# dmMaze/comic-text-detector

Measured on NVIDIA H100. Metric: pages/sec @1024x1024 synthetic, higher is better.
Workload: dtype fp16

## Files before the change

comic-text-detector_b200/csrc/conv_tc.cu:

```cuda
#include <cstdlib>
#include <cstring>
#include <cuda.h>
#include <cuda_fp16.h>
#include <cuda_runtime.h>

#include "kernels.h"
#include "ptx.cuh"

namespace ctd {

constexpr int kTileW = 16;
constexpr int kThreads = 384;

template <int BN, int TH>
struct TcCfg {
  static constexpr int kABytes = TH * kTileW * 128;
  static constexpr int kBBytes = BN * 128;
  static constexpr int kStages = TH == 8 ? (BN >= 128 ? 5 : (BN >= 64 ? 8 : 10))
                                         : (BN >= 128 ? 3 : (BN >= 64 ? 4 : (BN >= 32 ? 5 : 6)));
  static constexpr int kBoxN = BN < 64 ? BN : 64;
  static constexpr int kBoxBytes = 8 * TH * kBoxN * 2;
  static constexpr int kStgBytes = (BN / kBoxN) * kBoxBytes;
  static constexpr int kBiasFloats = 512;
  static constexpr size_t kSmem = 1024 + size_t(kStages) * (kABytes + kBBytes) + 2 * kStgBytes + 256 + kBiasFloats * 4;
// ... 61 lines not shown
  }
}

template <int ACT>
__device__ __forceinline__ void epi_pair_f32(float v0, float v1, const float* __restrict__ bias_s, int col,
                                             float* __restrict__ out, int ncols, bool residual) {
  if (col >= ncols) return;
  float f0 = apply_act_precise<ACT>(v0 + bias_s[col]);
  float f1 = apply_act_precise<ACT>(v1 + bias_s[col + 1]);
  if (col + 1 < ncols) {
    if (residual) {
      const float2 r = *reinterpret_cast<const float2*>(out + col);
      f0 += r.x;
      f1 += r.y;
    }
    *reinterpret_cast<float2*>(out + col) = make_float2(f0, f1);
  } else {
    if (residual) f0 += out[col];
    out[col] = f0;
  }
}

template <int BN, int ACT>
__device__ __forceinline__ void epilogue_f32(const float (&acc)[BN / 2], const float* __restrict__ bias_s,
                                             float* const (&out)[2], const bool (&valid)[2], int ncols, int lane,
                                             bool residual) {
#pragma unroll
  for (int h = 0; h < 2; ++h) {
    if (!valid[h]) continue;
#pragma unroll
    for (int j = 0; j < BN / 8; ++j)
      epi_pair_f32<ACT>(acc[j * 4 + 2 * h], acc[j * 4 + 2 * h + 1], bias_s, j * 8 + (lane & 3) * 2, out[h], ncols,
                        residual);
  }
}

template <int BN, int TH>
__global__ void __launch_bounds__(kThreads, 1) conv_tc_kernel(const __grid_constant__ ConvTcParams p) {
  using Cfg = TcCfg<BN, TH>;
  constexpr int MT = TH / 8;
  extern __shared__ __align__(1024) uint8_t smem_tc[];
  const uint32_t raw_base = smem_u32(smem_tc);
  const uint32_t smem_base = (raw_base + 1023u) & ~1023u;
  uint8_t* const smem_gen = smem_tc + (smem_base - raw_base);
  const uint32_t a_base = smem_base;
  const uint32_t b_base = a_base + Cfg::kStages * Cfg::kABytes;
  const uint32_t stg_base = b_base + Cfg::kStages * Cfg::kBBytes;
  const uint32_t bar_base = stg_base + 2 * Cfg::kStgBytes;
  const uint32_t full_bar = bar_base, empty_bar = bar_base + 8 * Cfg::kStages, res_bar0 = bar_base + 16 * Cfg::kStages;
  float* bias_s = reinterpret_cast<float*>(smem_gen + (bar_base - smem_base) + 256);

  const int warp = threadIdx.x >> 5, lane = threadIdx.x & 31;
  const ConvGeom& g = p.g;

  const int kb = p.kb_elems;
  const uint32_t row_bytes = kb * 2;
  const uint32_t stage_tx = uint32_t(TH * kTileW) * row_bytes + uint32_t(BN) * row_bytes;
  int kblocks_per_tap = 0;
  for (int s = 0; s < g.n_src; ++s) kblocks_per_tap += p.src_kblocks[s];
  const int n_terms = p.split ? 3 : 1;
  const int its_per_tile = g.taps * kblocks_per_tap * n_terms;
  const int tiles_per_img = p.tiles_x * p.tiles_y;
  const int n_nblk = g.cout_pad / BN;
  const int spatial_tiles = g.n_img * tiles_per_img;
  const int total_tiles = spatial_tiles * n_nblk * g.n_phase;

// ... 43 lines not shown
                const int stage = it % Cfg::kStages;
                const uint32_t par = ((it / Cfg::kStages) & 1) ^ 1;
                mbar_wait_relaxed(empty_bar + 8 * stage, par);
                mbar_arrive_expect_tx(full_bar + 8 * stage, stage_tx);
                tma_load_4d(a_base + stage * Cfg::kABytes, &p.a_map[s][q], full_bar + 8 * stage, cb * kb, x0 + dx,
                            y0 + dy, img + (term == 1 ? p.split_img_off : 0));
                tma_load_2d(b_base + stage * Cfg::kBBytes, &p.b_map, full_bar + 8 * stage, kglob + cb * kb,
                            phase * g.cout_pad + nblk * BN + (term == 2 ? p.split_row_off : 0));
              }
            }
            kglob += g.src_c[s];
          }
        }
      }
    }
    return;
  }

  if constexpr (TH == 16) setmaxnreg_inc<232>();
  const int wg = (warp >> 2) - 1;
  const int wrow = ((warp & 3) << 4) + (lane >> 2);
  const bool wg_leader = (threadIdx.x & 127) == 0;
  const uint64_t a_desc0 = make_kmajor_desc(a_base + uint32_t(wg * MT) * 64u * row_bytes, row_bytes);
  const uint64_t b_desc0 = make_kmajor_desc(b_base, row_bytes);
  const uint64_t a_mstep = (64u * row_bytes) >> 4;
  const int ksteps = kb / 16;
  int stage = 0;
  uint32_t full_par = 0;
  constexpr int R = BN / 2;
  const bool nhwc16 = p.dst != nullptr && !p.split;
  const bool res16 = nhwc16 && g.residual != 0;
  const uint32_t stg = stg_base + uint32_t(wg) * Cfg::kStgBytes;
  const uint32_t res_bar = res_bar0 + 8u * uint32_t(wg);
  const uint32_t epi_bar = 1 + wg;
  uint32_t res_par = 0;

  for (int t = blockIdx.x; t < total_tiles; t += gridDim.x) {
    int phase, nblk, img, y0, x0;
    decode(t, phase, nblk, img, y0, x0);
    const int sy0 = y0 + wg * (TH / 2);
    if (res16 && wg_leader) {
      tma_store_wait_read();
      mbar_arrive_expect_tx(res_bar, Cfg::kStgBytes);
#pragma unroll
      for (int b = 0; b < BN / Cfg::kBoxN; ++b)
        tma_load_4d(stg + b * Cfg::kBoxBytes, &p.d_map[phase], res_bar, nblk * BN + b * Cfg::kBoxN, x0, sy0, img);
    }
    float acc[MT][R];
#pragma unroll
    for (int m = 0; m < MT; ++m)
#pragma unroll
      for (int i = 0; i < R; ++i) acc[m][i] = 0.f;

    bool split_done = false;
    if constexpr (BN <= 64 && TH == 8) {
      if (p.split) {
        float cross[R], tmp[R];
#pragma unroll
        for (int i = 0; i < R; ++i) cross[i] = 0.f;
        bool cross_started = false;
        for (int k_it = 0; k_it < its_per_tile; ++k_it) {
          mbar_wait(full_bar + 8 * stage, full_par);
          const uint64_t ad = a_desc0 + uint64_t(stage) * (Cfg::kABytes >> 4);
          const uint64_t bd = b_desc0 + uint64_t(stage) * (Cfg::kBBytes >> 4);
          if (k_it % 3 == 0) {
            for (int ks = 0; ks < ksteps; ++ks) {
              wgmma_fence();
              wgmma_bn<BN>(tmp, ad + 2 * ks, bd + 2 * ks, 0u);
              wgmma_commit();
              wgmma_wait<0>();
              wgmma_fence_regs(tmp);
#pragma unroll
              for (int i = 0; i < R; ++i) acc[0][i] = __fadd_rn(acc[0][i], tmp[i]);
            }
          } else {
            wgmma_fence();
            for (int ks = 0; ks < ksteps; ++ks)
              wgmma_bn<BN>(cross, ad + 2 * ks, bd + 2 * ks, (cross_started || ks > 0) ? 1u : 0u);
            wgmma_commit();
            wgmma_wait<0>();
// ... 3 lines not shown
          if (wg_leader) mbar_arrive(empty_bar + 8 * stage);
          if (++stage == Cfg::kStages) { stage = 0; full_par ^= 1u; }
        }
#pragma unroll
        for (int i = 0; i < R; ++i) acc[0][i] = __fadd_rn(acc[0][i], cross[i] * kSplitLoUnscale);
        split_done = true;
      }
    }
    if (!split_done) {
      int prev = -1;
      for (int k_it = 0; k_it < its_per_tile; ++k_it) {
        mbar_wait(full_bar + 8 * stage, full_par);
        const uint64_t ad = a_desc0 + uint64_t(stage) * (Cfg::kABytes >> 4);
        const uint64_t bd = b_desc0 + uint64_t(stage) * (Cfg::kBBytes >> 4);
        wgmma_fence();
        for (int ks = 0; ks < ksteps; ++ks)
#pragma unroll
          for (int m = 0; m < MT; ++m)
            wgmma_bn<BN>(acc[m], ad + m * a_mstep + 2 * ks, bd + 2 * ks, (k_it > 0 || ks > 0) ? 1u : 0u);
        wgmma_commit();
        wgmma_wait<1>();
        if (prev >= 0 && wg_leader) mbar_arrive(empty_bar + 8 * prev);
        prev = stage;
        if (++stage == Cfg::kStages) { stage = 0; full_par ^= 1u; }
      }
      wgmma_wait<0>();
#pragma unroll
      for (int m = 0; m < MT; ++m) wgmma_fence_regs(acc[m]);
      if (prev >= 0 && wg_leader) mbar_arrive(empty_bar + 8 * prev);
    }

    const float* bias_t = bias_s + nblk * BN;
    if (nhwc16) {
      if (res16) {
        mbar_wait(res_bar, res_par);
        res_par ^= 1u;
      } else {
        if (wg_leader) tma_store_wait_read();
        named_barrier_sync(epi_bar, 128);
      }
#define CTD_EPI(ACT)                                                                                   \
  _Pragma("unroll") for (int m = 0; m < MT; ++m) {                                                     \
    if (res16) stage_f16<BN, TH, ACT, true>(acc[m], bias_t, stg, m, warp & 3, lane);                   \
    else stage_f16<BN, TH, ACT, false>(acc[m], bias_t, stg, m, warp & 3, lane);                        \
  }
      switch (g.act) {
        case CTD_ACT_SILU: CTD_EPI(CTD_ACT_SILU) break;
        case CTD_ACT_LEAKY: CTD_EPI(CTD_ACT_LEAKY) break;
        case CTD_ACT_RELU: CTD_EPI(CTD_ACT_RELU) break;
        case CTD_ACT_SIGMOID: CTD_EPI(CTD_ACT_SIGMOID) break;
        default: CTD_EPI(CTD_ACT_NONE) break;
      }
#undef CTD_EPI
      fence_proxy_async();
      named_barrier_sync(epi_bar, 128);
      if (wg_leader) {
#pragma unroll
        for (int b = 0; b < BN / Cfg::kBoxN; ++b)
          tma_store_4d(&p.d_map[phase], stg + b * Cfg::kBoxBytes, nblk * BN + b * Cfg::kBoxN, x0, sy0, img);
        tma_store_commit();
      }
      if (p.dst_map_cols < g.cout && p.dst_map_cols < (nblk + 1) * BN) {
#pragma unroll
        for (int m = 0; m < MT; ++m)
#pragma unroll
          for (int h = 0; h < 2; ++h) {
            const int row = (wg * MT + m) * 64 + wrow + 8 * h;
            const int gy = y0 + row / kTileW, gx = x0 + row % kTileW;
            if (gy >= g.gh || gx >= g.gw) continue;
            const int oy = gy * g.out_mul + (phase >> 1), ox = gx * g.out_mul + (phase & 1);
            __half* out = p.dst + (size_t(img) * g.dst_h * g.dst_w + size_t(oy) * g.dst_w + ox) * g.dst_cstride +
                          g.dst_coff;
#pragma unroll
            for (int i = 0; i < R; ++i) {
              if (((i >> 1) & 1) != h) continue;
              const int c = (i >> 2) * 8 + (lane & 3) * 2 + (i & 1), col = nblk * BN + c;
              if (col < p.dst_map_cols || col >= g.cout) continue;
              float f;
              switch (g.act) {
                case CTD_ACT_SILU: f = apply_act<CTD_ACT_SILU>(acc[m][i] + bias_t[c]); break;
                case CTD_ACT_LEAKY: f = apply_act<CTD_ACT_LEAKY>(acc[m][i] + bias_t[c]); break;
                case CTD_ACT_RELU: f = apply_act<CTD_ACT_RELU>(acc[m][i] + bias_t[c]); break;
                case CTD_ACT_SIGMOID: f = apply_act<CTD_ACT_SIGMOID>(acc[m][i] + bias_t[c]); break;
                default: f = acc[m][i] + bias_t[c]; break;
              }
              if (res16) f = __fadd_rn(f, __half2float(out[col]));
              out[col] = __float2half_rn(f);
            }
          }
      }
      continue;
    }
    const int ph_y = phase >> 1, ph_x = phase & 1;
    const int ncols = g.cout - nblk * BN;
#pragma unroll
    for (int m = 0; m < MT; ++m) {
      int gy[2], gx[2];
      bool valid[2];
      size_t pix[2];
#pragma unroll
      for (int h = 0; h < 2; ++h) {
        const int row = (wg * MT + m) * 64 + wrow + 8 * h;
        gy[h] = y0 + row / kTileW;
        gx[h] = x0 + row % kTileW;
        valid[h] = gy[h] < g.gh && gx[h] < g.gw;
        const int oy = gy[h] * g.out_mul + ph_y, ox = gx[h] * g.out_mul + ph_x;
        pix[h] = valid[h] ? size_t(img) * g.dst_h * g.dst_w + size_t(oy) * g.dst_w + ox : 0;
      }
      if (p.dst == nullptr) {
        const int no = 5 + p.nc;
        float* rows = p.blks + (size_t(img) * p.blks_rows_per_img + p.level_row0) * no;
#pragma unroll
        for (int h = 0; h < 2; ++h) {
          if (!valid[h]) continue;
#pragma unroll
          for (int i = 0; i < R; ++i) {
            if (((i >> 1) & 1) != h) continue;
            const int c = (i >> 2) * 8 + (lane & 3) * 2 + (i & 1);
            if (c >= ncols) continue;
            const int col = nblk * BN + c;
            const int a = col / no, o = col - a * no;
            const float s = 1.0f / (1.0f + expf(-(acc[m][i] + bias_t[c])));
            float r;
            if (o == 0) r = (s * 2.0f - 0.5f + float(gx[h])) * p.det_stride;
            else if (o == 1) r = (s * 2.0f - 0.5f + float(gy[h])) * p.det_stride;
            else if (o == 2) r = (s * 2.0f) * (s * 2.0f) * p.anchor_wh[2 * a];
            else if (o == 3) r = (s * 2.0f) * (s * 2.0f) * p.anchor_wh[2 * a + 1];
            else r = s;
            rows[(size_t(a) * g.gh * g.gw + size_t(gy[h]) * g.gw + gx[h]) * no + o] = r;
          }
        }
      } else {
        float* out32[2];
#pragma unroll
        for (int h = 0; h < 2; ++h)
          out32[h] = reinterpret_cast<float*>(p.dst) + pix[h] * g.dst_cstride + g.dst_coff + nblk * BN;
        const bool res = g.residual != 0;
        switch (g.act) {
          case CTD_ACT_SILU: epilogue_f32<BN, CTD_ACT_SILU>(acc[m], bias_t, out32, valid, ncols, lane, res); break;
          case CTD_ACT_LEAKY: epilogue_f32<BN, CTD_ACT_LEAKY>(acc[m], bias_t, out32, valid, ncols, lane, res); break;
          case CTD_ACT_RELU: epilogue_f32<BN, CTD_ACT_RELU>(acc[m], bias_t, out32, valid, ncols, lane, res); break;
          case CTD_ACT_SIGMOID: epilogue_f32<BN, CTD_ACT_SIGMOID>(acc[m], bias_t, out32, valid, ncols, lane, res); break;
          default: epilogue_f32<BN, CTD_ACT_NONE>(acc[m], bias_t, out32, valid, ncols, lane, res); break;
        }
      }
    }
  }
  if (nhwc16 && wg_leader) tma_store_wait_all();
}


static const char* encode_map(PFN_encodeTiled enc, CUtensorMap* m, const void* base, int rank, const cuuint64_t* dims,
                              const cuuint64_t* strides_bytes, const cuuint32_t* box, int kb_elems) {
  cuuint32_t estr[5] = {1, 1, 1, 1, 1};
  const CUtensorMapSwizzle sw = kb_elems == 64 ? CU_TENSOR_MAP_SWIZZLE_128B
                                               : (kb_elems == 32 ? CU_TENSOR_MAP_SWIZZLE_64B : CU_TENSOR_MAP_SWIZZLE_32B);
  CUresult r = enc(m, CU_TENSOR_MAP_DATA_TYPE_FLOAT16, rank, const_cast<void*>(base), dims, strides_bytes, box, estr,
                   CU_TENSOR_MAP_INTERLEAVE_NONE, sw, CU_TENSOR_MAP_L2_PROMOTION_L2_256B,
                   CU_TENSOR_MAP_FLOAT_OOB_FILL_NONE);
  return r == CUDA_SUCCESS ? nullptr : "cuTensorMapEncodeTiled failed";
}

static const char* encode_dst_maps(PFN_encodeTiled enc, ConvTcParams& p, const __half* dst, int bn, int th) {
  const ConvGeom& g = p.g;
  const int boxn = bn < 64 ? bn : 64;
  p.dst_map_cols = g.cout & ~7;
  if (p.dst_map_cols == 0) return "conv_tc: fp16 destination needs at least 8 output channels";
  const cuuint64_t px = cuuint64_t(g.dst_cstride) * 2;
  for (int ph = 0; ph < g.n_phase; ++ph) {
    const int ph_y = ph >> 1, ph_x = ph & 1;
    const char* base = reinterpret_cast<const char*>(dst) + size_t(g.dst_coff) * 2 + (size_t(ph_y) * g.dst_w + ph_x) * px;
    cuuint64_t dims[4] = {cuuint64_t(p.dst_map_cols), cuuint64_t(g.gw), cuuint64_t(g.gh), cuuint64_t(g.n_img)};
    cuuint64_t str[3] = {px * g.out_mul, px * g.dst_w * g.out_mul, px * g.dst_w * g.dst_h};
    cuuint32_t box[4] = {cuuint32_t(boxn), kTileW, cuuint32_t(th / 2), 1};
    if (const char* e = encode_map(enc, &p.d_map[ph], base, 4, dims, str, box, boxn)) return e;
  }
  return nullptr;
}

static int g_num_sms = 132;

// ... 49 lines not shown
  for (int s = 0; s < g.n_src; ++s) {
    const size_t cs = size_t(g.src_cstride[s]);
    const char* base = static_cast<const char*>(src_ptr[s]) + size_t(src_coff[s]) * 2;
    if (g.in_stride == 1) {
      cuuint64_t dims[4] = {cuuint64_t(g.src_c[s]), cuuint64_t(sw), cuuint64_t(sh), cuuint64_t(g.n_img * n_planes)};
      cuuint64_t str[3] = {cs * 2, cs * 2 * sw, cs * 2 * sw * sh};
      cuuint32_t box[4] = {cuuint32_t(kb), kTileW, cuuint32_t(th), 1};
      if (const char* e = encode_map(enc, &p.a_map[s][0], base, 4, dims, str, box, kb)) return e;
    } else {
      for (int q = 0; q < 4; ++q) {
        const int yp = q >> 1, xp = q & 1;
        cuuint64_t dims[4] = {cuuint64_t(g.src_c[s]), cuuint64_t(sw / 2), cuuint64_t(sh / 2), cuuint64_t(g.n_img * n_planes)};
        cuuint64_t str[3] = {cs * 2 * 2, cs * 2 * sw * 2, cs * 2 * sw * sh};
        cuuint32_t box[4] = {cuuint32_t(kb), kTileW, cuuint32_t(th), 1};
        const char* b2 = base + (size_t(yp) * sw + xp) * cs * 2;
        if (const char* e = encode_map(enc, &p.a_map[s][q], b2, 4, dims, str, box, kb)) return e;
      }
    }
  }
  for (int ph = 0; ph < g.n_phase; ++ph)
    for (int t = 0; t < g.taps; ++t) {
      if (g.in_stride == 2) {
        const int dy = g.tap_dy[ph][t], dx = g.tap_dx[ph][t];
        const int yp = dy != 0, xp = dx != 0;
        p.tap_map[ph][t] = int8_t(yp * 2 + xp);
        p.g.tap_dy[ph][t] = int8_t(dy < 0 ? -1 : 0);
        p.g.tap_dx[ph][t] = int8_t(dx < 0 ? -1 : 0);
      } else {
        p.tap_map[ph][t] = 0;
      }
    }
  plan.block_n = bn;
  plan.tile_h = th;
  if (dst != nullptr && !split)
    if (const char* e = encode_dst_maps(enc, p, dst, bn, th)) return e;
  if (split && ((g.dst_coff % 4) != 0 || (g.dst_cstride % 4) != 0 || (dst != nullptr && g.cout % 4 != 0)))
    return "conv_tc (split): fp32 destination slice must be 16-byte aligned";
  {
    cuuint64_t dims[2] = {cuuint64_t(g.k_total), cuuint64_t(g.n_phase) * cuuint64_t(g.cout_pad) * n_planes};
    cuuint64_t str[1] = {cuuint64_t(g.k_total) * 2};
    cuuint32_t box[2] = {cuuint32_t(kb), cuuint32_t(bn)};
    if (const char* e = encode_map(enc, &p.b_map, w16, 2, dims, str, box, kb)) return e;
  }
  {
    const int total_tiles = g.n_img * p.tiles_x * p.tiles_y * (g.cout_pad / bn) * g.n_phase;
    plan.grid = dim3(unsigned(total_tiles < g_num_sms ? total_tiles : g_num_sms), 1, 1);
  }
  if (g.cout_pad > 512) return "conv_tc: cout_pad > 512 not supported (bias staging)";
  plan.smem_bytes = th == 16 ? smem_for<16>(bn) : smem_for<8>(bn);
  return nullptr;
}

cudaError_t conv_tc_init() {
  cudaError_t e;
  int dev = 0;
  if (cudaGetDevice(&dev) == cudaSuccess) {
    int n = 0;
    if (cudaDeviceGetAttribute(&n, cudaDevAttrMultiProcessorCount, dev) == cudaSuccess && n > 0) g_num_sms = n;
  }
#define CTD_SET(BN, TH)                                                                                       \
  e = cudaFuncSetAttribute(conv_tc_kernel<BN, TH>, cudaFuncAttributeMaxDynamicSharedMemorySize,               \
                           int(TcCfg<BN, TH>::kSmem));                                                        \
  if (e != cudaSuccess) return e;
  CTD_SET(128, 8) CTD_SET(64, 8) CTD_SET(32, 8) CTD_SET(16, 8)
  CTD_SET(128, 16) CTD_SET(64, 16) CTD_SET(32, 16) CTD_SET(16, 16)
#undef CTD_SET
  return cudaSuccess;
}

template <int TH>
static void launch_th(const ConvTcPlan& plan, cudaStream_t s) {
  switch (plan.block_n) {
    case 128: conv_tc_kernel<128, TH><<<plan.grid, kThreads, plan.smem_bytes, s>>>(plan.p); break;
    case 64: conv_tc_kernel<64, TH><<<plan.grid, kThreads, plan.smem_bytes, s>>>(plan.p); break;
    case 32: conv_tc_kernel<32, TH><<<plan.grid, kThreads, plan.smem_bytes, s>>>(plan.p); break;
    default: conv_tc_kernel<16, TH><<<plan.grid, kThreads, plan.smem_bytes, s>>>(plan.p); break;
  }
}

cudaError_t conv_tc_launch(const ConvTcPlan& plan, cudaStream_t s) {
  if (plan.tile_h == 16) launch_th<16>(plan, s);
  else launch_th<8>(plan, s);
  return cudaGetLastError();
}

}
```

comic-text-detector_b200/csrc/engine.cu:

```cuda
#include <cuda.h>
#include <cuda_fp16.h>
#include <cuda_runtime.h>
#include <stdarg.h>
#include <stdio.h>
#include <string.h>

#include <algorithm>
#include <cstdlib>
#include <map>
#include <string>
#include <tuple>
#include <vector>

#include "engine.h"

using namespace ctd;

namespace {
thread_local std::string g_create_error;
}

int ctd_fail(ctd_handle* h, int code, const char* fmt, ...) {
  char buf[512];
  va_list ap;
// ... 278 lines not shown
static int build_plans(ctd_handle* h, int n, int ph, int pw, ShapePlan& sp) {
  sp.tc.resize(h->ops.size());
  sp.ends.resize(h->ops.size());
  const bool split = h->cfg.precision == CTD_PREC_SPLIT_TC;
  for (size_t i = 0; i < h->ops.size(); ++i) {
    const ctd_op& op = h->ops[i];
    if (!runs_on_tensor_cores(h->cfg.precision, op.kind)) continue;
    const float* bias = reinterpret_cast<const float*>(h->d_blob + op.b_off);
    const char* e = nullptr;
    if (op.kind == CTD_OP_STEM) {
      const bool f16 = sp.input == INPUT_F32;
      e = conv_ends_plan_stem(sp.ends[i], h->enc, f16 ? static_cast<const void*>(h->in_stage.p) : h->d_pages, f16, n,
                              ph, pw, h->d_blob + op.w16_off, bias, static_cast<__half*>(h->d_buf[op.dst_buf]),
                              h->bufs[op.dst_buf].channels, op.dst_coff, op.cout, op.act);
    } else if (op.kind == CTD_OP_SEG_TAIL) {
      if (op.cout_pad != 16) return ctd_fail(h, CTD_E_INVALID, "op %zu: seg tail needs cout_pad 16", i);
      const ctd_bufdesc& sb = h->bufs[op.src_buf[0]];
      e = conv_ends_plan_seg(sp.ends[i], h->enc, static_cast<const __half*>(h->d_buf[op.src_buf[0]]), sb.channels,
                             op.src_coff[0], op.src_c[0], n, ph / sb.down, pw / sb.down, h->d_blob + op.w16_off,
                             h->d_mask, h->d_mask_u8);
    } else {
      ConvGeom g;
      if (int rc = op_geom(h, op, n, ph, pw, g)) return rc;
      const void* src[CTD_MAX_SRC];
      int coff[CTD_MAX_SRC];
      for (int s = 0; s < op.n_src; ++s) {
        src[s] = (split ? h->d_buf16 : h->d_buf)[op.src_buf[s]];
        coff[s] = op.src_coff[s];
      }
      const void* w = split ? h->d_wsplit + h->wsplit_off[i] : h->d_blob + op.w16_off;
      __half* dst = op.kind == CTD_OP_DETECT ? nullptr : static_cast<__half*>(h->d_buf[op.dst_buf]);
      e = conv_tc_plan(sp.tc[i], h->enc, g, src, coff, w, bias, dst, split);
      if (op.kind == CTD_OP_DETECT) set_detect(h, i, ph, pw, sp.tc[i].p);
    }
    if (e) return ctd_fail(h, CTD_E_INVALID, "op %zu: %s", i, e);
  }
  return CTD_OK;
}

template <typename T>
static int run_op_simt(ctd_handle* h, size_t i, int n, int ph, int pw) {
  const ctd_op& op = h->ops[i];
  ConvSimtParams p;
  memset(&p, 0, sizeof(p));
  if (int rc = op_geom(h, op, n, ph, pw, p.g)) return rc;
  for (int k = 0; k < op.n_src; ++k)
    p.src[k] = static_cast<char*>(h->d_buf[op.src_buf[k]]) + size_t(op.src_coff[k]) * sizeof(T);
  p.w = h->d_blob + (sizeof(T) == 4 ? op.w32_off : op.w16_off);
  p.bias = reinterpret_cast<const float*>(h->d_blob + op.b_off);
  if (op.kind == CTD_OP_DETECT) set_detect(h, i, ph, pw, p);
  else p.dst = h->d_buf[op.dst_buf];
  CK(conv_simt_launch<T>(p, h->stream));
  return CTD_OK;
}

template <typename T>
static int run_op_thin(ctd_handle* h, const ctd_op& op, int n, int ph, int pw, int input) {
  cudaStream_t s = h->stream;
  const ctd_bufdesc* sb = op.kind == CTD_OP_STEM ? nullptr : &h->bufs[op.src_buf[0]];
  const int sh = sb ? ph / sb->down : ph, sw = sb ? pw / sb->down : pw;
  const T* src = sb ? static_cast<const T*>(h->d_buf[op.src_buf[0]]) + op.src_coff[0] : nullptr;
  switch (op.kind) {
    case CTD_OP_STEM: {
      const float* w = reinterpret_cast<const float*>(h->d_blob + op.w32_off);
      const float* b = reinterpret_cast<const float*>(h->d_blob + op.b_off);
      T* dst = static_cast<T*>(h->d_buf[op.dst_buf]);
// ... 666 lines not shown
```

comic-text-detector_b200/csrc/kernels.h:

```cpp
#pragma once
#include <cuda.h>
#include <cuda_fp16.h>
#include <cuda_runtime.h>
#include <stdint.h>

#include "../../include/ctd_b200.h"

namespace ctd {

constexpr int kMaxTaps = 9;

constexpr float kSplitLoScale = 2048.0f;
constexpr float kSplitLoUnscale = 1.0f / 2048.0f;
constexpr int kMaxPhases = 4;

struct ConvGeom {
  int n_img;
  int gh, gw;
  int dst_h, dst_w;
  int out_mul;
  int n_phase;
  int taps;
  int cin_total;
  int k_total;
// ... 9 lines not shown
  int act, residual;
};

void fill_conv_geom_taps(ConvGeom& g, int kind, int ksize, int stride);

struct alignas(64) ConvTcParams {
  CUtensorMap a_map[CTD_MAX_SRC][4];
  CUtensorMap b_map;
  CUtensorMap d_map[kMaxPhases];
  ConvGeom g;
  int kb_elems;
  int src_kblocks[CTD_MAX_SRC];
  int tiles_x, tiles_y;
  int8_t tap_map[kMaxPhases][kMaxTaps];
  __half* dst;
  int dst_map_cols;
  const float* bias;
  float* blks;
  int blks_rows_per_img;
  int level_row0;
  float det_stride;
  float anchor_wh[6];
  int nc;
  int split;
  int split_img_off;
  int split_row_off;
};
static_assert(sizeof(ConvTcParams) <= 4096, "ConvTcParams: kernel parameters are limited to 4 KB");

struct ConvTcPlan {
  ConvTcParams p;
  int block_n;
  int tile_h;
  dim3 grid;
  size_t smem_bytes;
};

typedef CUresult (*PFN_encodeTiled)(CUtensorMap*, CUtensorMapDataType, cuuint32_t, void*, const cuuint64_t*,
                                    const cuuint64_t*, const cuuint32_t*, const cuuint32_t*, CUtensorMapInterleave,
                                    CUtensorMapSwizzle, CUtensorMapL2promotion, CUtensorMapFloatOOBfill);

const char* conv_tc_plan(ConvTcPlan& plan, PFN_encodeTiled enc, const ConvGeom& g, const void* const src_ptr[],
                         const int src_coff[], const void* w16, const float* bias, __half* dst, int split = 0);
cudaError_t conv_tc_launch(const ConvTcPlan& plan, cudaStream_t s);
cudaError_t conv_tc_init();

enum { CTD_END_NONE = 0, CTD_END_STEM = 1, CTD_END_SEG = 2, CTD_END_STEM_F16 = 3 };
struct alignas(64) ConvEndsParams {
  CUtensorMap a_map;
  CUtensorMap b_map;
  CUtensorMap d_map;
  int n_img, gh, gw;
  int tiles_x, tiles_y;
  const float* bias;
  float* mask_f32;
  uint8_t* mask_u8;
};
struct ConvEndsPlan {
  ConvEndsParams p;
  int kind = CTD_END_NONE;
  dim3 grid;
  size_t smem_bytes;
};
const char* conv_ends_plan_stem(ConvEndsPlan& plan, PFN_encodeTiled enc, const void* pages, bool f16_page, int n,
                                int ph, int pw, const void* w16, const float* bias, __half* dst, int dst_cstride,
                                int dst_coff, int cout, int act);
const char* conv_ends_plan_seg(ConvEndsPlan& plan, PFN_encodeTiled enc, const __half* src, int src_cstride,
                               int src_coff, int src_c, int n, int gh, int gw, const void* w16, float* mask_f32,
                               uint8_t* mask_u8);
cudaError_t conv_ends_launch(const ConvEndsPlan& plan, cudaStream_t s);
cudaError_t conv_ends_init();

struct ConvSimtParams {
  ConvGeom g;
  const void* src[CTD_MAX_SRC];
  const void* w;
// ... 109 lines not shown
```

comic-text-detector_b200/csrc/ptx.cuh:

```cuda
#pragma once
#include <cuda_fp16.h>
#include <stdint.h>

namespace ctd {

__device__ __forceinline__ uint32_t smem_u32(const void* p) {
  return static_cast<uint32_t>(__cvta_generic_to_shared(p));
}

__device__ __forceinline__ bool elect_one() {
  uint32_t pred;
  asm volatile(
      "{\n"
      ".reg .pred P;\n"
      "elect.sync _|P, 0xffffffff;\n"
      "selp.b32 %0, 1, 0, P;\n"
      "}\n"
      : "=r"(pred));
  return pred != 0;
}

template <int N>
__device__ __forceinline__ void setmaxnreg_dec() { asm volatile("setmaxnreg.dec.sync.aligned.u32 %0;" ::"n"(N)); }
template <int N>
// ... 165 lines not shown
      "wgmma.mma_async.sync.aligned.m64n8k16.f32.f16.f16 "
      "{%0, %1, %2, %3}, "
      "{%4, %5, %6, %7}, %8, p, 1, 1, 0;\n"
      "}\n"
      : "+f"(d[0]), "+f"(d[1]), "+f"(d[2]), "+f"(d[3])
      : "r"(a[0]), "r"(a[1]), "r"(a[2]), "r"(a[3]), "l"(bdesc), "r"(accumulate));
}
__device__ __forceinline__ void wgmma_n16_rs(float (&d)[8], const uint32_t (&a)[4], uint64_t bdesc,
                                             uint32_t accumulate) {
  asm volatile(
      "{\n"
      ".reg .pred p;\n"
      "setp.ne.b32 p, %13, 0;\n"
      "wgmma.mma_async.sync.aligned.m64n16k16.f32.f16.f16 "
      "{%0, %1, %2, %3, %4, %5, %6, %7}, "
      "{%8, %9, %10, %11}, %12, p, 1, 1, 0;\n"
      "}\n"
      : "+f"(d[0]), "+f"(d[1]), "+f"(d[2]), "+f"(d[3]), "+f"(d[4]), "+f"(d[5]), "+f"(d[6]), "+f"(d[7])
      : "r"(a[0]), "r"(a[1]), "r"(a[2]), "r"(a[3]), "l"(bdesc), "r"(accumulate));
}
__device__ __forceinline__ void wgmma_n32_rs(float (&d)[16], const uint32_t (&a)[4], uint64_t bdesc,
                                             uint32_t accumulate) {
  asm volatile(
      "{\n"
      ".reg .pred p;\n"
      "setp.ne.b32 p, %21, 0;\n"
      "wgmma.mma_async.sync.aligned.m64n32k16.f32.f16.f16 "
      "{%0, %1, %2, %3, %4, %5, %6, %7, %8, %9, %10, %11, %12, %13, %14, %15}, "
      "{%16, %17, %18, %19}, %20, p, 1, 1, 0;\n"
      "}\n"
      : "+f"(d[0]), "+f"(d[1]), "+f"(d[2]), "+f"(d[3]), "+f"(d[4]), "+f"(d[5]), "+f"(d[6]), "+f"(d[7]), "+f"(d[8]), "+f"(d[9]), "+f"(d[10]), "+f"(d[11]), "+f"(d[12]), "+f"(d[13]), "+f"(d[14]), "+f"(d[15])
      : "r"(a[0]), "r"(a[1]), "r"(a[2]), "r"(a[3]), "l"(bdesc), "r"(accumulate));
}
template <int R>
__device__ __forceinline__ void wgmma_fence_regs(uint32_t (&a)[R]) {
#pragma unroll
  for (int i = 0; i < R; ++i) asm volatile("" : "+r"(a[i])::"memory");
}

__device__ __forceinline__ uint64_t make_kmajor_desc(uint32_t smem_addr, uint32_t swizzle_bytes) {
  const uint64_t layout = swizzle_bytes == 128 ? 1ull : (swizzle_bytes == 64 ? 2ull : 3ull);
  uint64_t d = 0;
  d |= static_cast<uint64_t>((smem_addr & 0x3FFFFu) >> 4);
  d |= 1ull << 16;
  d |= static_cast<uint64_t>((8u * swizzle_bytes) >> 4) << 32;
  d |= layout << 62;
  return d;
}

}
```

Before: 1131.

## Add halo-tile 3x3 conv kernel reusing one input slice across all nine taps

Adds a dedicated 3x3 stride-1 conv kernel. It TMA-loads one haloed input tile per channel block and builds the A operands for all nine taps from shared memory with ldmatrix, then feeds register-sourced wgmma. The previous path reloaded overlapping input data for each tap. When the weights fit, all nine tap weight blocks stay resident in shared memory. This adds many new template instantiations, more complex pipelining, and a routing path that could hit edge cases in slot or phase bookkeeping.

```diff
diff --git a/comic-text-detector_b200/csrc/conv_tc.cu b/comic-text-detector_b200/csrc/conv_tc.cu
--- a/comic-text-detector_b200/csrc/conv_tc.cu
+++ b/comic-text-detector_b200/csrc/conv_tc.cu
@@ -117,6 +117,87 @@
     for (int j = 0; j < BN / 8; ++j)
       epi_pair_f32<ACT>(acc[j * 4 + 2 * h], acc[j * 4 + 2 * h + 1], bias_s, j * 8 + (lane & 3) * 2, out[h], ncols,
                         residual);
+  }
+}
+
+template <int BN, int TH>
+__device__ __forceinline__ void load_residual(const ConvTcParams& p, uint32_t stg, uint32_t res_bar, int phase,
+                                              int nblk, int img, int x0, int sy0) {
+  using Cfg = TcCfg<BN, TH>;
+  tma_store_wait_read();
+  mbar_arrive_expect_tx(res_bar, Cfg::kStgBytes);
+#pragma unroll
+  for (int b = 0; b < BN / Cfg::kBoxN; ++b)
+    tma_load_4d(stg + b * Cfg::kBoxBytes, &p.d_map[phase], res_bar, nblk * BN + b * Cfg::kBoxN, x0, sy0, img);
+}
+
+template <int BN, int TH>
+__device__ __forceinline__ void epilogue_nhwc16(const ConvTcParams& p, const float (&acc)[TH / 8][BN / 2],
+                                                const float* __restrict__ bias_t, uint32_t stg, uint32_t res_bar,
+                                                uint32_t& res_par, bool res16, bool wg_leader, int wg, int warp,
+                                                int lane, int phase, int nblk, int img, int x0, int y0) {
+  using Cfg = TcCfg<BN, TH>;
+  constexpr int MT = TH / 8, R = BN / 2;
+  const ConvGeom& g = p.g;
+  const int sy0 = y0 + wg * (TH / 2);
+  const uint32_t epi_bar = 1 + wg;
+  if (res16) {
+    mbar_wait(res_bar, res_par);
+    res_par ^= 1u;
+  } else {
+    if (wg_leader) tma_store_wait_read();
+    named_barrier_sync(epi_bar, 128);
+  }
+#define CTD_EPI(ACT)                                                                                   \
+  _Pragma("unroll") for (int m = 0; m < MT; ++m) {                                                     \
+    if (res16) stage_f16<BN, TH, ACT, true>(acc[m], bias_t, stg, m, warp & 3, lane);                   \
+    else stage_f16<BN, TH, ACT, false>(acc[m], bias_t, stg, m, warp & 3, lane);                        \
+  }
+  switch (g.act) {
+    case CTD_ACT_SILU: CTD_EPI(CTD_ACT_SILU) break;
+    case CTD_ACT_LEAKY: CTD_EPI(CTD_ACT_LEAKY) break;
+    case CTD_ACT_RELU: CTD_EPI(CTD_ACT_RELU) break;
+    case CTD_ACT_SIGMOID: CTD_EPI(CTD_ACT_SIGMOID) break;
+    default: CTD_EPI(CTD_ACT_NONE) break;
+  }
+#undef CTD_EPI
+  fence_proxy_async();
+  named_barrier_sync(epi_bar, 128);
+  if (wg_leader) {
+#pragma unroll
+    for (int b = 0; b < BN / Cfg::kBoxN; ++b)
+      tma_store_4d(&p.d_map[phase], stg + b * Cfg::kBoxBytes, nblk * BN + b * Cfg::kBoxN, x0, sy0, img);
+    tma_store_commit();
+  }
+  if (p.dst_map_cols < g.cout && p.dst_map_cols < (nblk + 1) * BN) {
+    const int wrow = ((warp & 3) << 4) + (lane >> 2);
+#pragma unroll
+    for (int m = 0; m < MT; ++m)
+#pragma unroll
+      for (int h = 0; h < 2; ++h) {
+        const int row = (wg * MT + m) * 64 + wrow + 8 * h;
+        const int gy = y0 + row / kTileW, gx = x0 + row % kTileW;
+        if (gy >= g.gh || gx >= g.gw) continue;
+        const int oy = gy * g.out_mul + (phase >> 1), ox = gx * g.out_mul + (phase & 1);
+        __half* out = p.dst + (size_t(img) * g.dst_h * g.dst_w + size_t(oy) * g.dst_w + ox) * g.dst_cstride +
+                      g.dst_coff;
+#pragma unroll
+        for (int i = 0; i < R; ++i) {
+          if (((i >> 1) & 1) != h) continue;
+          const int c = (i >> 2) * 8 + (lane & 3) * 2 + (i & 1), col = nblk * BN + c;
+          if (col < p.dst_map_cols || col >= g.cout) continue;
+          float f;
+          switch (g.act) {
+            case CTD_ACT_SILU: f = apply_act<CTD_ACT_SILU>(acc[m][i] + bias_t[c]); break;
+            case CTD_ACT_LEAKY: f = apply_act<CTD_ACT_LEAKY>(acc[m][i] + bias_t[c]); break;
+            case CTD_ACT_RELU: f = apply_act<CTD_ACT_RELU>(acc[m][i] + bias_t[c]); break;
+            case CTD_ACT_SIGMOID: f = apply_act<CTD_ACT_SIGMOID>(acc[m][i] + bias_t[c]); break;
+            default: f = acc[m][i] + bias_t[c]; break;
+          }
+          if (res16) f = __fadd_rn(f, __half2float(out[col]));
+          out[col] = __float2half_rn(f);
+        }
+      }
   }
 }
 
@@ -226,20 +307,12 @@
   const bool res16 = nhwc16 && g.residual != 0;
   const uint32_t stg = stg_base + uint32_t(wg) * Cfg::kStgBytes;
   const uint32_t res_bar = res_bar0 + 8u * uint32_t(wg);
-  const uint32_t epi_bar = 1 + wg;
   uint32_t res_par = 0;
 
   for (int t = blockIdx.x; t < total_tiles; t += gridDim.x) {
     int phase, nblk, img, y0, x0;
     decode(t, phase, nblk, img, y0, x0);
-    const int sy0 = y0 + wg * (TH / 2);
-    if (res16 && wg_leader) {
-      tma_store_wait_read();
-      mbar_arrive_expect_tx(res_bar, Cfg::kStgBytes);
-#pragma unroll
-      for (int b = 0; b < BN / Cfg::kBoxN; ++b)
-        tma_load_4d(stg + b * Cfg::kBoxBytes, &p.d_map[phase], res_bar, nblk * BN + b * Cfg::kBoxN, x0, sy0, img);
-    }
+    if (res16 && wg_leader) load_residual<BN, TH>(p, stg, res_bar, phase, nblk, img, x0, y0 + wg * (TH / 2));
     float acc[MT][R];
 #pragma unroll
     for (int m = 0; m < MT; ++m)
@@ -309,63 +382,8 @@
 
     const float* bias_t = bias_s + nblk * BN;
     if (nhwc16) {
-      if (res16) {
-        mbar_wait(res_bar, res_par);
-        res_par ^= 1u;
-      } else {
-        if (wg_leader) tma_store_wait_read();
-        named_barrier_sync(epi_bar, 128);
-      }
-#define CTD_EPI(ACT)                                                                                   \
-  _Pragma("unroll") for (int m = 0; m < MT; ++m) {                                                     \
-    if (res16) stage_f16<BN, TH, ACT, true>(acc[m], bias_t, stg, m, warp & 3, lane);                   \
-    else stage_f16<BN, TH, ACT, false>(acc[m], bias_t, stg, m, warp & 3, lane);                        \
-  }
-      switch (g.act) {
-        case CTD_ACT_SILU: CTD_EPI(CTD_ACT_SILU) break;
-        case CTD_ACT_LEAKY: CTD_EPI(CTD_ACT_LEAKY) break;
-        case CTD_ACT_RELU: CTD_EPI(CTD_ACT_RELU) break;
-        case CTD_ACT_SIGMOID: CTD_EPI(CTD_ACT_SIGMOID) break;
-        default: CTD_EPI(CTD_ACT_NONE) break;
-      }
-#undef CTD_EPI
-      fence_proxy_async();
-      named_barrier_sync(epi_bar, 128);
-      if (wg_leader) {
-#pragma unroll
-        for (int b = 0; b < BN / Cfg::kBoxN; ++b)
-          tma_store_4d(&p.d_map[phase], stg + b * Cfg::kBoxBytes, nblk * BN + b * Cfg::kBoxN, x0, sy0, img);
-        tma_store_commit();
-      }
-      if (p.dst_map_cols < g.cout && p.dst_map_cols < (nblk + 1) * BN) {
-#pragma unroll
-        for (int m = 0; m < MT; ++m)
-#pragma unroll
-          for (int h = 0; h < 2; ++h) {
-            const int row = (wg * MT + m) * 64 + wrow + 8 * h;
-            const int gy = y0 + row / kTileW, gx = x0 + row % kTileW;
-            if (gy >= g.gh || gx >= g.gw) continue;
-            const int oy = gy * g.out_mul + (phase >> 1), ox = gx * g.out_mul + (phase & 1);
-            __half* out = p.dst + (size_t(img) * g.dst_h * g.dst_w + size_t(oy) * g.dst_w + ox) * g.dst_cstride +
-                          g.dst_coff;
-#pragma unroll
-            for (int i = 0; i < R; ++i) {
-              if (((i >> 1) & 1) != h) continue;
-              const int c = (i >> 2) * 8 + (lane & 3) * 2 + (i & 1), col = nblk * BN + c;
-              if (col < p.dst_map_cols || col >= g.cout) continue;
-              float f;
-              switch (g.act) {
-                case CTD_ACT_SILU: f = apply_act<CTD_ACT_SILU>(acc[m][i] + bias_t[c]); break;
-                case CTD_ACT_LEAKY: f = apply_act<CTD_ACT_LEAKY>(acc[m][i] + bias_t[c]); break;
-                case CTD_ACT_RELU: f = apply_act<CTD_ACT_RELU>(acc[m][i] + bias_t[c]); break;
-                case CTD_ACT_SIGMOID: f = apply_act<CTD_ACT_SIGMOID>(acc[m][i] + bias_t[c]); break;
-                default: f = acc[m][i] + bias_t[c]; break;
-              }
-              if (res16) f = __fadd_rn(f, __half2float(out[col]));
-              out[col] = __float2half_rn(f);
-            }
-          }
-      }
+      epilogue_nhwc16<BN, TH>(p, acc, bias_t, stg, res_bar, res_par, res16, wg_leader, wg, warp, lane, phase, nblk,
+                              img, x0, y0);
       continue;
     }
     const int ph_y = phase >> 1, ph_x = phase & 1;
@@ -424,6 +442,252 @@
     }
   }
   if (nhwc16 && wg_leader) tma_store_wait_all();
+}
+
+template <int BN, int TH, int KB, bool WR>
+struct Conv3Cfg {
+  using Tc = TcCfg<BN, TH>;
+  static constexpr int kHaloW = kTileW + 2, kHaloH = TH + 2;
+  static constexpr int kRowBytes = KB * 2;
+  static constexpr int kSliceTx = kHaloH * kHaloW * kRowBytes;
+  static constexpr int kSlotBytes = (kSliceTx + 1023) / 1024 * 1024;
+  static constexpr int kBStages = WR ? 9 : 4;
+  static constexpr int kBBytes = BN * kRowBytes;
+  static constexpr int kFixed = 1024 + kBStages * kBBytes + 2 * Tc::kStgBytes + 256 + Tc::kBiasFloats * 4;
+  static constexpr int kSmemMax = 227 * 1024;
+  static constexpr int kSlots = (kSmemMax - kFixed) / kSlotBytes < 8 ? (kSmemMax - kFixed) / kSlotBytes : 8;
+  static constexpr size_t kSmem = size_t(kFixed) + size_t(kSlots) * kSlotBytes;
+  static_assert(kSlots >= 1 && kSmem <= size_t(kSmemMax), "conv3_tc_kernel: shared memory");
+};
+
+template <int BN>
+__device__ __forceinline__ void wgmma_bn_rs(float (&d)[BN / 2], const uint32_t (&a)[4], uint64_t bd, uint32_t acc) {
+  if constexpr (BN == 128) wgmma_n128_rs(d, a, bd, acc);
+  else if constexpr (BN == 64) wgmma_n64_rs(d, a, bd, acc);
+  else if constexpr (BN == 32) wgmma_n32_rs(d, a, bd, acc);
+  else wgmma_n16_rs(d, a, bd, acc);
+}
+
+template <int BN, int TH, int KB, bool WR>
+__global__ void __launch_bounds__(kThreads, 1) conv3_tc_kernel(const __grid_constant__ ConvTcParams p) {
+  using Cfg = TcCfg<BN, TH>;
+  using C3 = Conv3Cfg<BN, TH, KB, WR>;
+  constexpr int MT = TH / 8;
+  constexpr int R = BN / 2;
+  constexpr int KS = KB / 16;
+  constexpr int G = BN * MT >= 256 ? 1 : KS * MT;
+  static_assert(!WR || (G > 1 && BN <= 64), "conv3_tc_kernel: resident weights take BN <= 64");
+  constexpr int S = C3::kSlots;
+  extern __shared__ __align__(1024) uint8_t smem_tc[];
+  const uint32_t raw_base = smem_u32(smem_tc);
+  const uint32_t smem_base = (raw_base + 1023u) & ~1023u;
+  uint8_t* const smem_gen = smem_tc + (smem_base - raw_base);
+  const uint32_t slice_base = smem_base;
+  const uint32_t b_base = slice_base + S * C3::kSlotBytes;
+  const uint32_t stg_base = b_base + C3::kBStages * C3::kBBytes;
+  const uint32_t bar_base = stg_base + 2 * Cfg::kStgBytes;
+  const uint32_t bfull = bar_base, bempty = bar_base + 32, sfull = bar_base + 64, sempty = bar_base + 128,
+                 res_bar0 = bar_base + 192;
+  float* bias_s = reinterpret_cast<float*>(smem_gen + (bar_base - smem_base) + 256);
+
+  const int warp = threadIdx.x >> 5, lane = threadIdx.x & 31;
+  const ConvGeom& g = p.g;
+  int nkb = 0;
+  for (int s = 0; s < g.n_src; ++s) nkb += p.src_kblocks[s];
+  const int tiles_per_img = p.tiles_x * p.tiles_y;
+  const int n_nblk = g.cout_pad / BN;
+  const int total_tiles = g.n_img * tiles_per_img * n_nblk;
+
+  if (warp == 0 && lane == 0) {
+    for (int s = 0; s < g.n_src; ++s) prefetch_tensormap(&p.a_map[s][0]);
+    prefetch_tensormap(&p.b_map);
+    prefetch_tensormap(&p.d_map[0]);
+    for (int s = 0; s < (WR ? 1 : C3::kBStages); ++s) {
+      mbar_init(bfull + 8 * s, 1);
+      mbar_init(bempty + 8 * s, 2);
+    }
+    for (int s = 0; s < S; ++s) {
+      mbar_init(sfull + 8 * s, 1);
+      mbar_init(sempty + 8 * s, 8);
+    }
+    mbar_init(res_bar0, 1);
+    mbar_init(res_bar0 + 8, 1);
+    fence_barrier_init();
+  }
+  for (int i = threadIdx.x; i < g.cout_pad && i < Cfg::kBiasFloats; i += kThreads) bias_s[i] = p.bias ? p.bias[i] : 0.f;
+  __syncthreads();
+
+  auto decode = [&](int t, int& nblk, int& img, int& y0, int& x0) {
+    nblk = t % n_nblk;
+    const int sp = t / n_nblk;
+    img = sp / tiles_per_img;
+    const int trem = sp - img * tiles_per_img;
+    const int ty = trem / p.tiles_x;
+    y0 = ty * TH;
+    x0 = (trem - ty * p.tiles_x) * kTileW;
+  };
+
+  if (warp < 4) {
+    if constexpr (TH == 16) setmaxnreg_dec<40>();
+    if (warp == 0 && elect_one()) {
+      int slot = 0, stage = 0;
+      uint32_t spar = 1, bpar = 1;
+      if constexpr (WR) {
+        mbar_arrive_expect_tx(bfull, 9 * C3::kBBytes);
+        for (int tap = 0; tap < 9; ++tap)
+          tma_load_2d(b_base + tap * C3::kBBytes, &p.b_map, bfull, tap * g.cin_total, 0);
+      }
+      for (int t = blockIdx.x; t < total_tiles; t += gridDim.x) {
+        int nblk, img, y0, x0;
+        decode(t, nblk, img, y0, x0);
+        for (int tap = 0; tap < (WR ? 1 : 9); ++tap) {
+          int kglob = tap * g.cin_total;
+          for (int s = 0; s < g.n_src; ++s) {
+            for (int cb = 0; cb < p.src_kblocks[s]; ++cb) {
+              if (tap == 0) {
+                mbar_wait_relaxed(sempty + 8 * slot, spar);
+                mbar_arrive_expect_tx(sfull + 8 * slot, C3::kSliceTx);
+                tma_load_4d(slice_base + slot * C3::kSlotBytes, &p.a_map[s][0], sfull + 8 * slot, cb * KB, x0 - 1,
+                            y0 - 1, img);
+                if (++slot == S) { slot = 0; spar ^= 1u; }
+              }
+              if constexpr (WR) continue;
+              mbar_wait_relaxed(bempty + 8 * stage, bpar);
+              mbar_arrive_expect_tx(bfull + 8 * stage, C3::kBBytes);
+              tma_load_2d(b_base + stage * C3::kBBytes, &p.b_map, bfull + 8 * stage, kglob + cb * KB, nblk * BN);
+              if (++stage == C3::kBStages) { stage = 0; bpar ^= 1u; }
+            }
+            kglob += g.src_c[s];
+          }
+        }
+      }
+    }
+    return;
+  }
+
+  if constexpr (TH == 16) setmaxnreg_inc<232>();
+  const int wg = (warp >> 2) - 1;
+  const bool wg_leader = (threadIdx.x & 127) == 0;
+  const bool res16 = g.residual != 0;
+  const uint32_t stg = stg_base + uint32_t(wg) * Cfg::kStgBytes;
+  const uint32_t res_bar = res_bar0 + 8u * uint32_t(wg);
+  const int q = lane >> 3;
+  const int lpix = (4 * wg * MT + (warp & 3)) * C3::kHaloW + (lane & 7) + 8 * (q & 1);
+  int bstage = 0, seq = 0;
+  uint32_t bpar = 0, res_par = 0;
+  if constexpr (WR) mbar_wait(bfull, 0);
+
+  for (int t = blockIdx.x; t < total_tiles; t += gridDim.x) {
+    if (res16 && wg_leader) {
+      int nblk, img, y0, x0;
+      decode(t, nblk, img, y0, x0);
+      load_residual<BN, TH>(p, stg, res_bar, 0, nblk, img, x0, y0 + wg * (TH / 2));
+    }
+    float acc[MT][R];
+#pragma unroll
+    for (int m = 0; m < MT; ++m)
+#pragma unroll
+      for (int i = 0; i < R; ++i) acc[m][i] = 0.f;
+
+    const int slot0 = seq % S;
+    auto slot_of = [&](int cb) { return slot0 + cb < S ? slot0 + cb : slot0 + cb - S; };
+    auto load_a = [&](int tap, int cb, int ks, int m, uint32_t (&frag)[4]) {
+      const int slot = slot_of(cb);
+      const int dy = tap / 3, dx = tap - 3 * dy;
+      const uint32_t off = uint32_t(lpix + (4 * m + dy) * C3::kHaloW + dx) * C3::kRowBytes + (2 * ks + (q >> 1)) * 16;
+      ldmatrix_x4(slice_base + uint32_t(slot) * C3::kSlotBytes + (off ^ (((off >> 7) & (C3::kRowBytes / 16 - 1)) << 4)),
+                  frag);
+      if (tap == 8 && ks == KS - 1 && m == MT - 1) {
+        __syncwarp();
+        if (lane == 0) mbar_arrive(sempty + 8 * slot);
+      }
+    };
+    auto load_group = [&](int tap, int cb, uint32_t (&set)[G][4]) {
+#pragma unroll
+      for (int u = 0; u < G; ++u) load_a(tap, cb, u / MT, u % MT, set[u]);
+    };
+
+    uint32_t a[2][G][4];
+    mbar_wait(sfull + 8 * slot0, (seq / S) & 1);
+    load_group(0, 0, a[0]);
+    int prev_stage = -1;
+    if constexpr (G == 1) {
+      for (int tap = 0; tap < 9; ++tap) {
+        for (int cb = 0; cb < nkb; ++cb) {
+          int ntap = tap, ncb = cb + 1;
+          if (ncb == nkb) { ncb = 0; ++ntap; }
+          if (ntap == 0) mbar_wait(sfull + 8 * slot_of(ncb), ((seq + ncb) / S) & 1);
+          mbar_wait(bfull + 8 * bstage, bpar);
+          const uint64_t bd = make_kmajor_desc(b_base + uint32_t(bstage) * C3::kBBytes, C3::kRowBytes);
+          const bool first = tap == 0 && cb == 0;
+#pragma unroll
+          for (int i = 0; i < KS * MT; ++i) {
+            const int ks = i / MT, m = i % MT;
+            wgmma_fence();
+            wgmma_bn_rs<BN>(acc[m], a[i & 1][0], bd + 2 * ks, (first && ks == 0) ? 0u : 1u);
+            wgmma_commit();
+            wgmma_wait<1>();
+            if (i == 0 && prev_stage >= 0 && wg_leader) mbar_arrive(bempty + 8 * prev_stage);
+            if (i + 1 < KS * MT) {
+              wgmma_fence_regs(a[(i + 1) & 1][0]);
+              load_a(tap, cb, (i + 1) / MT, (i + 1) % MT, a[(i + 1) & 1][0]);
+            } else if (ntap < 9) {
+              wgmma_fence_regs(a[0][0]);
+              load_a(ntap, ncb, 0, 0, a[0][0]);
+            }
+          }
+          prev_stage = bstage;
+          if (++bstage == C3::kBStages) { bstage = 0; bpar ^= 1u; }
+        }
+      }
+    } else {
+      int tap = 0, cb = 0;
+      auto kblock = [&](bool first, bool last, uint32_t (&cur)[G][4], uint32_t (&nxt)[G][4]) {
+        int ntap = tap, ncb = cb + 1;
+        if (ncb == nkb) { ncb = 0; ++ntap; }
+        if (ntap == 0) mbar_wait(sfull + 8 * slot_of(ncb), ((seq + ncb) / S) & 1);
+        if constexpr (!WR) mbar_wait(bfull + 8 * bstage, bpar);
+        const uint64_t bd = make_kmajor_desc(b_base + uint32_t(WR ? tap : bstage) * C3::kBBytes, C3::kRowBytes);
+        wgmma_fence();
+#pragma unroll
+        for (int u = 0; u < G; ++u)
+          wgmma_bn_rs<BN>(acc[u % MT], cur[u], bd + 2 * (u / MT), (first && u < MT) ? 0u : 1u);
+        wgmma_commit();
+        wgmma_wait<1>();
+        if (!WR && prev_stage >= 0 && wg_leader) mbar_arrive(bempty + 8 * prev_stage);
+#pragma unroll
+        for (int u = 0; u < G; ++u) wgmma_fence_regs(nxt[u]);
+        if (!last) load_group(ntap, ncb, nxt);
+        if constexpr (!WR) {
+          prev_stage = bstage;
+          if (++bstage == C3::kBStages) { bstage = 0; bpar ^= 1u; }
+        }
+        tap = ntap;
+        cb = ncb;
+      };
+      const int nblocks = 9 * nkb;
+      for (int kk = 0; kk < nblocks; kk += 2) {
+        kblock(kk == 0, kk + 1 == nblocks, a[0], a[1]);
+        if (kk + 1 < nblocks) kblock(false, kk + 2 == nblocks, a[1], a[0]);
+      }
+    }
+    wgmma_wait<0>();
+#pragma unroll
+    for (int m = 0; m < MT; ++m) wgmma_fence_regs(acc[m]);
+#pragma unroll
+    for (int u = 0; u < G; ++u) {
+      wgmma_fence_regs(a[0][u]);
+      wgmma_fence_regs(a[1][u]);
+    }
+    if (!WR && wg_leader) mbar_arrive(bempty + 8 * prev_stage);
+    seq += nkb;
+
+    int nblk, img, y0, x0;
+    decode(t, nblk, img, y0, x0);
+    epilogue_nhwc16<BN, TH>(p, acc, bias_s + nblk * BN, stg, res_bar, res_par, res16, wg_leader, wg, warp, lane, 0,
+                            nblk, img, x0, y0);
+  }
+  if (wg_leader) tma_store_wait_all();
 }
 
 
@@ -539,6 +803,7 @@
     }
   plan.block_n = bn;
   plan.tile_h = th;
+  plan.halo = 0;
   if (dst != nullptr && !split)
     if (const char* e = encode_dst_maps(enc, p, dst, bn, th)) return e;
   if (split && ((g.dst_coff % 4) != 0 || (g.dst_cstride % 4) != 0 || (dst != nullptr && g.cout % 4 != 0)))
@@ -558,6 +823,50 @@
   return nullptr;
 }
 
+template <int TH, int KB, bool WR>
+static void conv3_cfg(int bn, int& slots, size_t& smem) {
+#define CTD_CFG(BN) { slots = Conv3Cfg<BN, TH, KB, WR>::kSlots; smem = Conv3Cfg<BN, TH, KB, WR>::kSmem; }
+  switch (bn) {
+    case 128: if constexpr (!WR) CTD_CFG(128) break;
+    case 64: CTD_CFG(64) break;
+    case 32: CTD_CFG(32) break;
+    default: CTD_CFG(16) break;
+  }
+#undef CTD_CFG
+}
+
+const char* conv3_tc_route(ConvTcPlan& plan, PFN_encodeTiled enc, const void* const src_ptr[], const int src_coff[]) {
+  ConvTcParams& p = plan.p;
+  const ConvGeom& g = p.g;
+  plan.halo = 0;
+  if (p.split || p.dst == nullptr || g.n_phase != 1 || g.taps != 9 || g.in_stride != 1 || p.kb_elems < 32)
+    return nullptr;
+  const int th = plan.tile_h, bn = plan.block_n, kb = p.kb_elems;
+  int slots = 0, nkb = 0;
+  size_t smem = 0;
+  for (int s = 0; s < g.n_src; ++s) nkb += p.src_kblocks[s];
+  const bool wr = nkb == 1 && g.cout_pad == bn && bn <= 64;
+  if (wr) {
+    if (th == 16) kb == 64 ? conv3_cfg<16, 64, true>(bn, slots, smem) : conv3_cfg<16, 32, true>(bn, slots, smem);
+    else kb == 64 ? conv3_cfg<8, 64, true>(bn, slots, smem) : conv3_cfg<8, 32, true>(bn, slots, smem);
+  } else {
+    if (th == 16) kb == 64 ? conv3_cfg<16, 64, false>(bn, slots, smem) : conv3_cfg<16, 32, false>(bn, slots, smem);
+    else kb == 64 ? conv3_cfg<8, 64, false>(bn, slots, smem) : conv3_cfg<8, 32, false>(bn, slots, smem);
+  }
+  if (slots < nkb) return nullptr;
+  for (int s = 0; s < g.n_src; ++s) {
+    const size_t cs = size_t(g.src_cstride[s]);
+    const char* base = static_cast<const char*>(src_ptr[s]) + size_t(src_coff[s]) * 2;
+    cuuint64_t dims[4] = {cuuint64_t(g.src_c[s]), cuuint64_t(g.src_w), cuuint64_t(g.src_h), cuuint64_t(g.n_img)};
+    cuuint64_t str[3] = {cs * 2, cs * 2 * g.src_w, cs * 2 * g.src_w * g.src_h};
+    cuuint32_t box[4] = {cuuint32_t(kb), kTileW + 2, cuuint32_t(th + 2), 1};
+    if (const char* e = encode_map(enc, &p.a_map[s][0], base, 4, dims, str, box, kb)) return e;
+  }
+  plan.halo = wr ? 2 : 1;
+  plan.smem_bytes = smem;
+  return nullptr;
+}
+
 cudaError_t conv_tc_init() {
   cudaError_t e;
   int dev = 0;
@@ -572,11 +881,46 @@
   CTD_SET(128, 8) CTD_SET(64, 8) CTD_SET(32, 8) CTD_SET(16, 8)
   CTD_SET(128, 16) CTD_SET(64, 16) CTD_SET(32, 16) CTD_SET(16, 16)
 #undef CTD_SET
+#define CTD_SET(BN, TH, KB, WR)                                                                               \
+  e = cudaFuncSetAttribute(conv3_tc_kernel<BN, TH, KB, WR>, cudaFuncAttributeMaxDynamicSharedMemorySize,      \
+                           int(Conv3Cfg<BN, TH, KB, WR>::kSmem));                                             \
+  if (e != cudaSuccess) return e;
+#define CTD_SET_BN(TH, KB)                                                                                    \
+  CTD_SET(128, TH, KB, false) CTD_SET(64, TH, KB, false) CTD_SET(32, TH, KB, false) CTD_SET(16, TH, KB, false) \
+  CTD_SET(64, TH, KB, true) CTD_SET(32, TH, KB, true) CTD_SET(16, TH, KB, true)
+  CTD_SET_BN(8, 64) CTD_SET_BN(8, 32) CTD_SET_BN(16, 64) CTD_SET_BN(16, 32)
+#undef CTD_SET_BN
+#undef CTD_SET
   return cudaSuccess;
+}
+
+template <int TH, int KB>
+static void launch_conv3(const ConvTcPlan& plan, cudaStream_t s) {
+#define CTD_L(BN, WR) conv3_tc_kernel<BN, TH, KB, WR><<<plan.grid, kThreads, plan.smem_bytes, s>>>(plan.p)
+  if (plan.halo == 2) {
+    switch (plan.block_n) {
+      case 64: CTD_L(64, true); break;
+      case 32: CTD_L(32, true); break;
+      default: CTD_L(16, true); break;
+    }
+    return;
+  }
+  switch (plan.block_n) {
+    case 128: CTD_L(128, false); break;
+    case 64: CTD_L(64, false); break;
+    case 32: CTD_L(32, false); break;
+    default: CTD_L(16, false); break;
+  }
+#undef CTD_L
 }
 
 template <int TH>
 static void launch_th(const ConvTcPlan& plan, cudaStream_t s) {
+  if (plan.halo) {
+    if (plan.p.kb_elems == 64) launch_conv3<TH, 64>(plan, s);
+    else launch_conv3<TH, 32>(plan, s);
+    return;
+  }
   switch (plan.block_n) {
     case 128: conv_tc_kernel<128, TH><<<plan.grid, kThreads, plan.smem_bytes, s>>>(plan.p); break;
     case 64: conv_tc_kernel<64, TH><<<plan.grid, kThreads, plan.smem_bytes, s>>>(plan.p); break;
diff --git a/comic-text-detector_b200/csrc/engine.cu b/comic-text-detector_b200/csrc/engine.cu
--- a/comic-text-detector_b200/csrc/engine.cu
+++ b/comic-text-detector_b200/csrc/engine.cu
@@ -334,6 +334,7 @@
       __half* dst = op.kind == CTD_OP_DETECT ? nullptr : static_cast<__half*>(h->d_buf[op.dst_buf]);
       e = conv_tc_plan(sp.tc[i], h->enc, g, src, coff, w, bias, dst, split);
       if (op.kind == CTD_OP_DETECT) set_detect(h, i, ph, pw, sp.tc[i].p);
+      else if (!e && op.kind == CTD_OP_CONV) e = conv3_tc_route(sp.tc[i], h->enc, src, coff);
     }
     if (e) return ctd_fail(h, CTD_E_INVALID, "op %zu: %s", i, e);
   }
diff --git a/comic-text-detector_b200/csrc/kernels.h b/comic-text-detector_b200/csrc/kernels.h
--- a/comic-text-detector_b200/csrc/kernels.h
+++ b/comic-text-detector_b200/csrc/kernels.h
@@ -65,6 +65,7 @@
   ConvTcParams p;
   int block_n;
   int tile_h;
+  int halo;
   dim3 grid;
   size_t smem_bytes;
 };
@@ -75,6 +76,7 @@
 
 const char* conv_tc_plan(ConvTcPlan& plan, PFN_encodeTiled enc, const ConvGeom& g, const void* const src_ptr[],
                          const int src_coff[], const void* w16, const float* bias, __half* dst, int split = 0);
+const char* conv3_tc_route(ConvTcPlan& plan, PFN_encodeTiled enc, const void* const src_ptr[], const int src_coff[]);
 cudaError_t conv_tc_launch(const ConvTcPlan& plan, cudaStream_t s);
 cudaError_t conv_tc_init();
 
diff --git a/comic-text-detector_b200/csrc/ptx.cuh b/comic-text-detector_b200/csrc/ptx.cuh
--- a/comic-text-detector_b200/csrc/ptx.cuh
+++ b/comic-text-detector_b200/csrc/ptx.cuh
@@ -221,6 +221,32 @@
       : "+f"(d[0]), "+f"(d[1]), "+f"(d[2]), "+f"(d[3]), "+f"(d[4]), "+f"(d[5]), "+f"(d[6]), "+f"(d[7]), "+f"(d[8]), "+f"(d[9]), "+f"(d[10]), "+f"(d[11]), "+f"(d[12]), "+f"(d[13]), "+f"(d[14]), "+f"(d[15])
       : "r"(a[0]), "r"(a[1]), "r"(a[2]), "r"(a[3]), "l"(bdesc), "r"(accumulate));
 }
+__device__ __forceinline__ void wgmma_n64_rs(float (&d)[32], const uint32_t (&a)[4], uint64_t bdesc,
+                                             uint32_t accumulate) {
+  asm volatile(
+      "{\n"
+      ".reg .pred p;\n"
+      "setp.ne.b32 p, %37, 0;\n"
+      "wgmma.mma_async.sync.aligned.m64n64k16.f32.f16.f16 "
+      "{%0, %1, %2, %3, %4, %5, %6, %7, %8, %9, %10, %11, %12, %13, %14, %15, %16, %17, %18, %19, %20, %21, %22, %23, %24, %25, %26, %27, %28, %29, %30, %31}, "
+      "{%32, %33, %34, %35}, %36, p, 1, 1, 0;\n"
+      "}\n"
+      : "+f"(d[0]), "+f"(d[1]), "+f"(d[2]), "+f"(d[3]), "+f"(d[4]), "+f"(d[5]), "+f"(d[6]), "+f"(d[7]), "+f"(d[8]), "+f"(d[9]), "+f"(d[10]), "+f"(d[11]), "+f"(d[12]), "+f"(d[13]), "+f"(d[14]), "+f"(d[15]), "+f"(d[16]), "+f"(d[17]), "+f"(d[18]), "+f"(d[19]), "+f"(d[20]), "+f"(d[21]), "+f"(d[22]), "+f"(d[23]), "+f"(d[24]), "+f"(d[25]), "+f"(d[26]), "+f"(d[27]), "+f"(d[28]), "+f"(d[29]), "+f"(d[30]), "+f"(d[31])
+      : "r"(a[0]), "r"(a[1]), "r"(a[2]), "r"(a[3]), "l"(bdesc), "r"(accumulate));
+}
+__device__ __forceinline__ void wgmma_n128_rs(float (&d)[64], const uint32_t (&a)[4], uint64_t bdesc,
+                                              uint32_t accumulate) {
+  asm volatile(
+      "{\n"
+      ".reg .pred p;\n"
+      "setp.ne.b32 p, %69, 0;\n"
+      "wgmma.mma_async.sync.aligned.m64n128k16.f32.f16.f16 "
+      "{%0, %1, %2, %3, %4, %5, %6, %7, %8, %9, %10, %11, %12, %13, %14, %15, %16, %17, %18, %19, %20, %21, %22, %23, %24, %25, %26, %27, %28, %29, %30, %31, %32, %33, %34, %35, %36, %37, %38, %39, %40, %41, %42, %43, %44, %45, %46, %47, %48, %49, %50, %51, %52, %53, %54, %55, %56, %57, %58, %59, %60, %61, %62, %63}, "
+      "{%64, %65, %66, %67}, %68, p, 1, 1, 0;\n"
+      "}\n"
+      : "+f"(d[0]), "+f"(d[1]), "+f"(d[2]), "+f"(d[3]), "+f"(d[4]), "+f"(d[5]), "+f"(d[6]), "+f"(d[7]), "+f"(d[8]), "+f"(d[9]), "+f"(d[10]), "+f"(d[11]), "+f"(d[12]), "+f"(d[13]), "+f"(d[14]), "+f"(d[15]), "+f"(d[16]), "+f"(d[17]), "+f"(d[18]), "+f"(d[19]), "+f"(d[20]), "+f"(d[21]), "+f"(d[22]), "+f"(d[23]), "+f"(d[24]), "+f"(d[25]), "+f"(d[26]), "+f"(d[27]), "+f"(d[28]), "+f"(d[29]), "+f"(d[30]), "+f"(d[31]), "+f"(d[32]), "+f"(d[33]), "+f"(d[34]), "+f"(d[35]), "+f"(d[36]), "+f"(d[37]), "+f"(d[38]), "+f"(d[39]), "+f"(d[40]), "+f"(d[41]), "+f"(d[42]), "+f"(d[43]), "+f"(d[44]), "+f"(d[45]), "+f"(d[46]), "+f"(d[47]), "+f"(d[48]), "+f"(d[49]), "+f"(d[50]), "+f"(d[51]), "+f"(d[52]), "+f"(d[53]), "+f"(d[54]), "+f"(d[55]), "+f"(d[56]), "+f"(d[57]), "+f"(d[58]), "+f"(d[59]), "+f"(d[60]), "+f"(d[61]), "+f"(d[62]), "+f"(d[63])
+      : "r"(a[0]), "r"(a[1]), "r"(a[2]), "r"(a[3]), "l"(bdesc), "r"(accumulate));
+}
 template <int R>
 __device__ __forceinline__ void wgmma_fence_regs(uint32_t (&a)[R]) {
 #pragma unroll
```

Measured after the change: 1137 (median of 6 runs). No clear change (+0.5%).
